# tsai0507/PolishPathPlanning

Hardware: AMD Instinct MI355X
Metric: polishing waypoints/sec for 1M-pt cloud, 256 slices; path L2 err vs ref (higher is better)
Workload: dtype f32; 1 GPU; cfg2_1m_s256; points_per_workpiece=999912, slices=256, waypoints_per_workpiece=25908, workpieces=1, batch_per_gpu=1, parallelism=single GPU, pairing=kd, walk=center_int (connect), dynamic_adjustment=False, handles_taking_turns=3

## Files before the change

polishpathplanning_amd/csrc/ppp_engine.hip:

```cpp
#include "ppp_kernels.h"
#ifdef PPP_SINGLE_TU
#include "ppp_window.h"
#else
#include "ppp_window_decl.h"
#endif
#include "ppp_preproc.h"
#include "ppp_sort.h"
#include "ppp_align.h"
#include "ppp_gather.h"
#include <atomic>
#include <cerrno>
#include <fcntl.h>
#include <thread>
#include <unistd.h>
#ifndef PPP_NN_HINT_SPACINGS
#define PPP_NN_HINT_SPACINGS 3.0
#endif
#ifndef PPP_SLAB_PTS
#define PPP_SLAB_PTS 832
#endif
#ifndef PPP_PPT8_FROM
#define PPP_PPT8_FROM 500000
#endif
#ifndef WIN_SLICE_WAVES_PER_CU
// ... 139 lines not shown
    DevBuf<int> wp_cnt, wp_off, tail, slice_wpcnt;
    DevBuf<float4> wp_xyz, wp_normal;
    DevBuf<int> wp_nn;
    DevBuf<float> wp_pre, wp_smooth, wp_out;
    DevBuf<MinMaxPart> mm_part;
    DevBuf<int> big_slabs, big_slices;
    DevBuf<char> arena;
    bool big_path = false;
    int mm_grid = 1, mm_grid_used = 1, sm_tiles = 1;
    DevBuf<char> scratch;
    bool win_allowed = true;
    bool win_disabled = false;
    bool win_path = false;
    bool win_staged = false;
    bool stage_compact = true;
    float win_pad = 4.f;
    int win_NBc_thr = 0;
    int win_capw = 0, win_cap_el = 0, win_NB = 0, win_NBc = 0, win_stride = 1, win_threads = 256, win_ppt = 4, win_gs = 1;
    int win_rec_lds = 0;
    int win_nkept = 0, win_first_kept = 0, win_el_expect = 0;
    float win_px0 = 0.f;
    DevBuf<float> win_px;
    DevBuf<int> win_cnt;
    DevBuf<float4> win_pts;
    DevBuf<MinMaxPart> win_part;
    DevBuf<float4> wps_xyz, wps_normal, wps_rec;
    DevBuf<int> fin_ticket;
    DevBuf<int> wps_nn;
    DevBuf<float> wps_pre;

// ... 417 lines not shown
    memset(&A, 0, sizeof(A));
    A.m = h->meta.p; A.P = dev_params(h);
    A.X = h->use_part ? h->Xp.p : h->X.p; A.Y = h->use_part ? h->Yp.p : h->Y.p; A.Z = h->use_part ? h->Zp.p : h->Z.p;
    A.idmap = h->use_part ? h->part_idx.p : ((h->part_given && h->part_has_idx) ? h->part_idx.p : nullptr);
    A.n = h->use_part ? h->n_part : (int)h->n;
    A.plan_px = h->win_px.p;
    A.S = h->S_cap; A.sb = h->sb; A.se = h->se; A.first_kept = h->win_first_kept; A.nkept = h->win_nkept;
    A.pad = h->win_pad; A.px0 = h->win_px0; A.inv_step = 1.0f / (float)std::max(1, (int)(h->P.tool_radius * 2));
    A.y0 = h->h_mn[1];
    { const float yr = h->h_mx[1] - h->h_mn[1]; A.yscale = yr > 0.f ? (float)h->win_NBc / yr : 0.f; }
    for (int d = 0; d < 3; ++d) { A.plan_mn[d] = h->h_mn[d]; A.plan_mx[d] = h->h_mx[d]; }
    A.plan_nvalid = h->h_nvalid;
    A.capw = h->win_capw; A.cap_el = h->win_cap_el; A.NB = h->win_NB; A.NBc = h->win_NBc; A.stride = h->win_stride; A.rec_lds = h->win_rec_lds;
    A.W_cap = h->W_cap; A.node_cap = h->node_cap;
    A.g_scatter = h->win_gs; A.g_slice = std::max(0, h->se - h->sb); A.g_finish = h->sm_tiles;
    A.finish = h->ranged ? 0 : 1;
    A.win_cnt = h->win_cnt.p; A.win_pts = h->win_pts.p; A.win_part = h->win_part.p;
    A.px = h->px.p; A.lo = h->lo.p; A.hi = h->hi.p;
    A.node_x = h->node_x.p; A.node_y = h->node_y.p; A.node_z = h->node_z.p;
    A.node_start = h->node_start.p; A.node_cnt = h->node_cnt.p; A.band_cnt = h->band_cnt.p;
    A.wp_cnt = h->wp_cnt.p; A.wp_off = h->wp_off.p; A.tail = h->tail.p;
    A.wps_xyz = h->wps_xyz.p; A.wps_normal = h->wps_normal.p; A.wps_nn = h->wps_nn.p; A.wps_pre = h->wps_pre.p; A.wps_rec = h->wps_rec.p;
    A.wp_pre = h->wp_pre.p; A.wp_smooth = h->wp_smooth.p; A.wp_out = h->wp_out.p; A.out2 = h->out2; A.out2_cap = h->out2_cap;
    A.plan_rec = (h->rec_current && h->plan_walk_ok) ? h->plan_auto.p : nullptr;
    A.meta_host = h->hmeta_pinned.p; A.fin_ticket = h->fin_ticket.p;
    return A;
}
size_t win_slice_lds(const ppp_handle h) { return win_slice_lds_for(h, h->win_NBc); }
void win_args_throughput(const ppp_handle h, WinArgs &A)
{
    A.NBc = h->win_NBc_thr; A.NB = WIN_CLASSES * A.NBc;
// ... 14 lines not shown
    else LAUNCH(h, "k_win_scatter", (k_win_scatter<4, false>), A.g_scatter, WSC_T, scat_lds, A);
    const int T = h->win_threads;
    const size_t lds = win_slice_lds_for(h, A.NBc);
    const int extra = tuning_env("PPP_WIN_NO_VERIFY") ? 0 : 1;
    if (T <= 256) LAUNCH(h, "k_win_slice", k_win_slice<256>, A.g_slice + extra, T, lds, A);
    else if (T <= 512) LAUNCH(h, "k_win_slice", k_win_slice<512>, A.g_slice + extra, T, lds, A);
    else if (T <= 768) LAUNCH(h, "k_win_slice", k_win_slice<768>, A.g_slice + extra, T, lds, A);
    else LAUNCH(h, "k_win_slice", k_win_slice<1024>, A.g_slice + extra, T, lds, A);
    h->stage_compact = false;
    return PPP_OK;
}
int enqueue_window_finish(ppp_handle h)
{
    const WinArgs A = win_args(h);
    LAUNCH(h, "k_win_finish", k_win_finish, A.g_finish, SMF_T, sizeof(int) * ((size_t)A.nkept + 2), A);
    return PPP_OK;
}

template <class Sel>
int compact(ppp_handle h, Sel &sel, int n, int *cnt, int *total, const std::function<int(int)> &sized = nullptr)
{
    const int nblocks = (n + COMPACT_CHUNK - 1) / COMPACT_CHUNK;
    LAUNCH(h, "k_compact_count", k_compact_count<Sel>, nblocks, 256, 0, sel, n, cnt);
    LAUNCH(h, "k_compact_scan", k_compact_scan, 1, 1024, 0, cnt, nblocks, total);
    if (sized) {
        int kept = 0;
        HIPCHK(h, hipMemcpyAsync(&kept, total, sizeof(int), hipMemcpyDeviceToHost, h->stream));
        HIPCHK(h, hipStreamSynchronize(h->stream));
        if (int rc = sized(kept)) return rc;
    }
// ... 114 lines not shown
        h->dyn_maxNB = (int)std::min(4.0e6, std::max(0.0, yr - 4) / (h->P.tool_radius / 4) + 4);
        h->dyn_maxNA = (int)std::min(4.0e6, yr / 5 + 4);
        h->node_cap = (int)std::min(2.0e9, (double)h->node_cap + (double)h->S_cap * h->dyn_maxNA);
        int rc = ensure_dynamic_buffers(h);
        if (rc) return rc;
    }
    HIPCHK(h, h->node_x.ensure(h->node_cap)); HIPCHK(h, h->node_y.ensure(h->node_cap)); HIPCHK(h, h->node_z.ensure(h->node_cap));
    HIPCHK(h, h->node_start.ensure(h->S_cap)); HIPCHK(h, h->node_cnt.ensure(h->S_cap)); HIPCHK(h, h->band_cnt.ensure(h->S_cap));
    HIPCHK(h, h->wp_cnt.ensure(h->S_cap)); HIPCHK(h, h->wp_off.ensure(h->S_cap + 1)); HIPCHK(h, h->tail.ensure(h->S_cap));
    HIPCHK(h, h->slice_wpcnt.ensure(h->S_cap));
    HIPCHK(h, h->wp_xyz.ensure(h->W_cap)); HIPCHK(h, h->wp_normal.ensure(h->W_cap)); HIPCHK(h, h->wp_nn.ensure(h->W_cap));
    HIPCHK(h, h->wp_pre.ensure(6 * (size_t)h->W_cap)); HIPCHK(h, h->wp_smooth.ensure(6 * (size_t)h->W_cap));
    HIPCHK(h, h->wp_out.ensure(6 * (size_t)h->W_cap));
    h->sm_tiles = smooth_tiles(h->W_cap);
    { int rcw = plan_window(h, S, per); if (rcw) return rcw; }
    h->stage_compact = true;
    h->planned = true;
    h->index_built = false; h->gen_done = false; h->meta_fresh = false; h->path_done = false; h->list_final = false;
    h->drop_graph();
    return PPP_OK;
}

int slice_threads(const ppp_handle h, long long slices_in_launch)
{
    const bool two_fit = 2 * (slice_kd_bytes(h->capb) + 1024) <= (size_t)h->max_lds;
    return (two_fit && slices_in_launch >= 2LL * h->num_cus) ? 512 : SLICE_KD_T;
}

int enqueue_index(ppp_handle h)
{
    const int n = h->use_part ? h->n_part : (int)h->n;
// ... 416 lines not shown
const char *ppp_version(void) { return PPP_VERSION_STR; }

int ppp_create(int device_id, ppp_handle *out)
{
    if (!out) return PPP_ERR_ARG;
    *out = nullptr;
    int count = 0;
    if (hipGetDeviceCount(&count) != hipSuccess || count <= 0) return PPP_ERR_NO_DEVICE;
    if (device_id < 0 || device_id >= count) return PPP_ERR_ARG;
    if (hipSetDevice(device_id) != hipSuccess) return PPP_ERR_HIP;
    ppp_handle h = new ppp_handle_s();
    h->device = device_id;
    ppp_default_params(&h->P);
    if (hipStreamCreateWithFlags(&h->stream, hipStreamNonBlocking) != hipSuccess) { delete h; return PPP_ERR_HIP; }
    if (h->meta.ensure(1) != hipSuccess) { delete h; return PPP_ERR_HIP; }
    if (hipMemset(h->meta.p, 0, sizeof(DevMeta)) != hipSuccess) { delete h; return PPP_ERR_HIP; }
    if (h->fin_ticket.ensure(1 + WIN_FIN_GROUPS) != hipSuccess || hipMemset(h->fin_ticket.p, 0, sizeof(int) * (1 + WIN_FIN_GROUPS)) != hipSuccess) { delete h; return PPP_ERR_HIP; }
    if (h->hmeta_pinned.ensure(1) != hipSuccess) { delete h; return PPP_ERR_HIP; }
    int lds = 0;
    if (hipDeviceGetAttribute(&lds, hipDeviceAttributeMaxSharedMemoryPerBlock, device_id) == hipSuccess && lds > 0) h->max_lds = lds;
    hipDeviceProp_t prop;
    if (hipGetDeviceProperties(&prop, device_id) == hipSuccess) {
        if (strncmp(prop.gcnArchName, "gfx950", 6) == 0) h->max_lds = std::max(h->max_lds, 160 * 1024);
        if (prop.multiProcessorCount > 0) h->num_cus = prop.multiProcessorCount;
    }
    (void)hipFuncSetAttribute((const void *)k_slice, hipFuncAttributeMaxDynamicSharedMemorySize, h->max_lds - 1024);
    (void)hipFuncSetAttribute((const void *)k_slice_kd<false>, hipFuncAttributeMaxDynamicSharedMemorySize, h->max_lds - 1024);
    (void)hipFuncSetAttribute((const void *)k_minmax<true>, hipFuncAttributeMaxDynamicSharedMemorySize, 16384 * 4);
    (void)hipFuncSetAttribute((const void *)k_slab_scatter<0, 4>, hipFuncAttributeMaxDynamicSharedMemorySize, 16384 * 4);
    (void)hipFuncSetAttribute((const void *)k_slab_scatter<0, 8>, hipFuncAttributeMaxDynamicSharedMemorySize, 16384 * 4);
    (void)hipFuncSetAttribute((const void *)k_slab_scatter<1, 8>, hipFuncAttributeMaxDynamicSharedMemorySize, 16384 * 4);
    (void)hipFuncSetAttribute((const void *)k_slab_scatter<2, 4>, hipFuncAttributeMaxDynamicSharedMemorySize, 16384 * 4);
// ... 633 lines not shown
               h->wp_xyz.p, h->wp_nn.p, h->wp_normal.p, h->wp_pre.p, PB, h->slab_ytab.p, cnt_in);
    } else
    {
#define PPP_POSE_ARGS h->meta.p, D, h->sorted4.p, h->slab_start.p, h->slab_xmin.p, \
           h->slab_xmax.p, h->px.p, h->node_x.p, h->node_y.p, h->node_z.p, h->node_start.p, h->node_cnt.p, h->wp_cnt.p, h->wp_off.p, \
           h->tail.p, h->W_cap, h->big_path ? 1 : 0, h->knot_cap, h->stage_cap, h->tab_slabs, h->pose_pad, \
           h->wp_xyz.p, h->wp_nn.p, h->wp_normal.p, h->wp_pre.p, PB, h->slab_ytab.p, cnt_in
        if (h->pose_threads <= 256) LAUNCH(h, "k_pose", (k_pose<false, 256>), nk, h->pose_threads, pose_lds_bytes(h->knot_cap, h->stage_cap, h->tab_slabs), PPP_POSE_ARGS);
        else if (h->pose_threads <= 512) LAUNCH(h, "k_pose", (k_pose<false, 512>), nk, h->pose_threads, pose_lds_bytes(h->knot_cap, h->stage_cap, h->tab_slabs), PPP_POSE_ARGS);
        else if (h->pose_threads <= 768) LAUNCH(h, "k_pose", (k_pose<false, 768>), nk, h->pose_threads, pose_lds_bytes(h->knot_cap, h->stage_cap, h->tab_slabs), PPP_POSE_ARGS);
        else LAUNCH(h, "k_pose", (k_pose<false, POSE_T>), nk, h->pose_threads, pose_lds_bytes(h->knot_cap, h->stage_cap, h->tab_slabs), PPP_POSE_ARGS);
#undef PPP_POSE_ARGS
    }
    h->path_done = true;
    h->list_final = false;
    h->stage_compact = true;
    if (!h->ranged) {
        int rc = enqueue_finish(h, D);
        if (rc) return rc;
        h->list_final = true;
        return PPP_OK;
    }
    return enqueue_meta_copy(h);
}

int ppp_finish_path_async(ppp_handle h, const float *pre6_dev, size_t W, const int *counts, size_t nkept)
{
    if (!h) return PPP_ERR_ARG;
    HIPCHK(h, hipSetDevice(h->device));
    { int rcs = settle(h); if (rcs) return rcs; }
    if (!h->have_cloud) return fail(h, PPP_ERR_ARG, "no cloud set");
    if (!h->planned) { int rc = make_plan(h); if (rc) return rc; }
    if ((W && !pre6_dev) || (nkept && !counts)) return fail(h, PPP_ERR_ARG, "bad arguments");
    if (W > (size_t)h->W_cap || nkept > (size_t)h->S_cap) return fail(h, PPP_ERR_CAPACITY, "the list is larger than this handle's plan (other cloud or parameters?)");
    if (!h->index_built && !h->win_path) { int rc = enqueue_index(h); if (rc) return rc; }
    DevParams D = dev_params(h);
    if (nkept) HIPCHK(h, hipMemcpyAsync(h->wp_cnt.p, counts, nkept * sizeof(int), hipMemcpyHostToDevice, h->stream));
    LAUNCH(h, "k_count_given", k_count_given, 1, 1024, 0, h->meta.p, D, (int)nkept, (int)W, h->wp_cnt.p, h->wp_off.p, h->tail.p, h->W_cap);
    if (W) LAUNCH(h, "k_load_pre", k_load_pre, (unsigned)((W + 255) / 256), 256, 0, h->meta.p, pre6_dev, h->wp_pre.p);
    int rc = enqueue_finish(h, D);
    if (rc) return rc;
    h->gen_done = true; ++h->gen_serial; h->path_done = true; h->list_final = true;
    h->stage_compact = true;
    return PPP_OK;
}

int ppp_run_async(ppp_handle h)
{
    if (!h) return PPP_ERR_ARG;
    HIPCHK(h, hipSetDevice(h->device));
    { int rcs = settle_enqueue_only(h); if (rcs) return rcs; }
    if (!h->have_cloud) return fail(h, PPP_ERR_ARG, "no cloud set");
    if (!h->planned) { int rc = make_plan(h); if (rc) return rc; }
    h->last_out2 = nullptr; h->last_out2_cap = 0;
    if (h->timing) {
        int rc = ppp_gen_path_async(h);
        return rc ? rc : ppp_get_path_async(h);
    }
// ... 15 lines not shown
        h->chain_calls = false;
        if (rc == PPP_OK) rc = ppp_get_path_async(h);
        --h->internal;
        hipGraph_t g = nullptr;
        hipError_t e = hipStreamEndCapture(h->stream, &g);
        if (rc != PPP_OK) { if (g) (void)hipGraphDestroy(g); return rc; }
        if (e != hipSuccess) return fail(h, PPP_ERR_HIP, std::string("hipStreamEndCapture: ") + hipGetErrorString(e));
        h->graph = g;
        e = hipGraphInstantiate(&h->graph_exec, h->graph, nullptr, nullptr, 0);
        if (e != hipSuccess) { h->drop_graph(); return fail(h, PPP_ERR_HIP, std::string("hipGraphInstantiate: ") + hipGetErrorString(e)); }
    }
    h->meta_fresh = false;
    HIPCHK(h, hipGraphLaunch(h->graph_exec, h->stream));
    if (!h->win_path) h->index_built = true;
    h->stage_compact = !h->win_path;
    h->gen_done = true; ++h->gen_serial; h->path_done = true;
    h->list_final = !h->ranged;
    h->meta_in_flight = true;
    h->meta_from_batch = false;
    return PPP_OK;
}

extern "C++" {
namespace {

bool batch_eligible(const ppp_handle h)
{
    return h->P.pairing == PPP_PAIR_KD && !h->P.dynamic_adjustment && !h->aligned && !h->ranged && !h->big_path && !h->two_pass_scatter &&
           slice_lds_ok(h, h->capb);
}
// ... 304 lines not shown
                return fail(lead, PPP_ERR_HIP, std::string("batch capture (") + where + "): " + hipGetErrorString(e != hipSuccess ? e : e2));
            }
            bg->g = g;
            e = hipGraphInstantiate(&bg->ge, bg->g, nullptr, nullptr, 0);
            if (e != hipSuccess) { discard(); return fail(lead, PPP_ERR_HIP, std::string("hipGraphInstantiate: ") + hipGetErrorString(e)); }
        }
        bg->epochs.resize(count);
        for (size_t i = 0; i < count; ++i) bg->epochs[i] = hs[i]->epoch;
    }
    if (bg->eager) { int rc = enqueue_batched(lead, bg); if (rc) return rc; }
    else HIPCHK(lead, hipGraphLaunch(bg->ge, lead->stream));
    for (size_t i = 0; i < count; ++i) {
        ppp_handle h = hs[i];
        if (!(bg->batched && bg->win) && !(!bg->batched && h->win_path)) h->index_built = true;
        h->stage_compact = !((bg->batched && bg->win) || (!bg->batched && h->win_path));
        h->gen_done = true; ++h->gen_serial; h->path_done = true;
        h->list_final = !h->ranged;
        h->meta_fresh = false;
        h->meta_in_flight = !(bg->batched && count == 1);
        h->meta_from_batch = bg->batched && count > 1;
        if (bg->batched && count > 1) { h->bmetas = bg->hmetas; h->bslot = i; }
        h->pending_stream = (i == 0) ? nullptr : lead->stream;
        remember_dst(i);
    }
    return PPP_OK;
}

extern "C++" {
namespace {
struct Rccl {
// ... 181 lines not shown
int ppp_get_waypoint_counts(ppp_handle h, int *counts, size_t cap, size_t *nkept)
{
    int rc = ensure_ready(h, true, true);
    if (rc) return rc;
    rc = map_dev_err(h);
    if (rc) return rc;
    size_t nk = (size_t)h->hmeta.nkept;
    if (nkept) *nkept = nk;
    if (counts && cap) {
        size_t k = std::min(cap, nk);
        if (k) HIPCHK(h, copy_sync(h, counts, h->wp_cnt.p, k * sizeof(int), hipMemcpyDeviceToHost));
    }
    return PPP_OK;
}

int ppp_copy_stage_to_device(ppp_handle h, int stage, float *dst_dev, size_t cap, size_t *W)
{
    int rc = ensure_ready(h, true, true);
    if (rc) return rc;
    rc = map_dev_err(h);
    if (rc) return rc;
    const float *src = stage == PPP_STAGE_WP_PRESMOOTH ? h->wp_pre.p : stage == PPP_STAGE_WP_SMOOTHED ? h->wp_smooth.p : nullptr;
    if (!src) return fail(h, PPP_ERR_ARG, "stage must be PPP_STAGE_WP_PRESMOOTH or PPP_STAGE_WP_SMOOTHED");
    if (stage == PPP_STAGE_WP_SMOOTHED && !h->list_final) return fail(h, PPP_ERR_ARG, NOT_FINAL_MSG);
    size_t w = (size_t)h->hmeta.W;
    if (W) *W = w;
    size_t k = std::min(cap, w);
    if (k && dst_dev) {
        HIPCHK(h, hipMemcpyAsync(dst_dev, src, k * 24, hipMemcpyDeviceToDevice, h->stream));
        HIPCHK(h, hipStreamSynchronize(h->stream));
    }
    return PPP_OK;
}

static int bounds_ready(ppp_handle h)
{
    if (h && h->have_cloud && h->planned && h->win_path && h->gen_done) {
        HIPCHK(h, hipSetDevice(h->device));
        return PPP_OK;
// ... 453 lines not shown
           h->slab_xmax.p, dq, (int)k, dout);
    HIPCHK(h, hipMemcpyAsync(idx, dout, k * 4, hipMemcpyDeviceToHost, h->stream));
    HIPCHK(h, hipStreamSynchronize(h->stream));
    return PPP_OK;
}

static int ensure_stage_lists(ppp_handle h)
{
    if (h->stage_compact || !h->win_path) return PPP_OK;
    const WinArgs A = win_args(h);
    if (A.nkept > 0) LAUNCH(h, "k_win_gather_stage", k_win_gather_stage, A.nkept, 256, 0, A, h->wp_xyz.p, h->wp_nn.p, h->wp_normal.p);
    h->stage_compact = true;
    return PPP_OK;
}

int ppp_get_stage(ppp_handle h, int stage, void *out, size_t cap_bytes, size_t *count)
{
    int rc = ensure_ready(h, true, true);
    if (rc) return rc;
    rc = map_dev_err(h);
    if (rc) return rc;
    if (stage == PPP_STAGE_WP_XYZ || stage == PPP_STAGE_WP_NN || stage == PPP_STAGE_WP_NORMAL) { rc = ensure_stage_lists(h); if (rc) return rc; }
    size_t W = (size_t)h->hmeta.W;
    if (count) *count = W;
    if (!out || !cap_bytes || !W) return PPP_OK;
    const void *src = nullptr;
    size_t elem = 0;
    std::vector<float> tmp;
    switch (stage) {
    case PPP_STAGE_WP_XYZ: {
        std::vector<float4> t4(W);
        HIPCHK(h, copy_sync(h, t4.data(), h->wp_xyz.p, W * 16, hipMemcpyDeviceToHost));
        tmp.resize(3 * W);
        for (size_t i = 0; i < W; ++i) { tmp[3 * i] = t4[i].x; tmp[3 * i + 1] = t4[i].y; tmp[3 * i + 2] = t4[i].z; }
        memcpy(out, tmp.data(), std::min(cap_bytes, W * 12));
        return PPP_OK;
    }
// ... 198 lines not shown
```

polishpathplanning_amd/csrc/ppp_window.h:

```cpp
#pragma once
#include "ppp_kernels.h"
#include "ppp_window_decl.h"

template <int PPT, bool STAGED>
__device__ __forceinline__ void win_scatter_body(const WinArgs &A, const int bx)
{
    extern __shared__ __attribute__((aligned(16))) int s_dyn[];
    float *s_px = (float *)s_dyn;
    int *s_cnt = s_dyn + A.S;
    __shared__ int s_scr[17];
    __shared__ float s_mn[3][WSC_T / 64], s_mx[3][WSC_T / 64];
    __shared__ int s_n[WSC_T / 64];
    const int S = A.S, n = A.n;
    const int i0 = bx * (PPT * (int)blockDim.x);
    STAMP_BEGIN();
    float4 p[PPT];
#pragma unroll
    for (int k = 0; k < PPT; ++k) {
        const int i = i0 + threadIdx.x + k * (int)blockDim.x;
        if (i < n) p[k] = make_float4(A.X[i], A.Y[i], A.Z[i], __int_as_float(A.idmap ? A.idmap[i] : i));
        else p[k] = make_float4(NAN, 0.f, 0.f, 0.f);
    }
    for (int s = threadIdx.x; s < S; s += blockDim.x) { s_px[s] = A.plan_px[s]; s_cnt[s] = 0; }
    if (bx == 0 && threadIdx.x == 0) {
        DevMeta *m = A.m;
        m->W = 0; m->err = 0; m->err_slice = 0x7fffffff; m->sweeps = 0; m->any_short = 0; m->rpy_oob = 0;
        m->node_cursor = 0; m->smooth_done = -1; m->emit_ticket = 0; m->big_slabs = 0; m->big_slices = 0; m->arena_cursor = 0; m->win_flag = 0;
        if (A.fin_ticket) for (int q = 0; q <= WIN_FIN_GROUPS; ++q) A.fin_ticket[q] = 0;
    }
    __syncthreads();
    STAMP(7, 0);
    float mn[3] = {INFINITY, INFINITY, INFINITY}, mx[3] = {-INFINITY, -INFINITY, -INFINITY};
    int cnt = 0;
    int pw[PPT], pr[PPT];
#pragma unroll
    for (int k = 0; k < PPT; ++k) {
        const float x = p[k].x;
        pw[k] = -1; pr[k] = 0;
        if (x == x) {
            mn[0] = fminf(mn[0], x); mx[0] = fmaxf(mx[0], x);
            mn[1] = fminf(mn[1], p[k].y); mx[1] = fmaxf(mx[1], p[k].y);
            mn[2] = fminf(mn[2], p[k].z); mx[2] = fmaxf(mx[2], p[k].z);
            cnt++;
            const float fj = fminf(fmaxf(floorf((x - s_px[0]) * A.inv_step + 0.5f), 0.f), (float)(S - 1));
            const int j = (int)fj;
            const int ja = j > 0 ? j - 1 : j, jb = j + 1 < S ? j + 1 : j;
            const float da = fabsf(x - s_px[ja]), dj = fabsf(x - s_px[j]), db = fabsf(x - s_px[jb]);
            int w = -1;
            if (dj <= A.pad) w = j; else if (da <= A.pad) w = ja; else if (db <= A.pad) w = jb;
            if (w >= A.sb && w < A.se) { pw[k] = w; pr[k] = atomicAdd(&s_cnt[w], 1); }
        }
    }
    __syncthreads();
    STAMP(7, 1);
    if (!STAGED) {
        for (int s = threadIdx.x; s < S; s += blockDim.x) {
            const int c = s_cnt[s];
            if (c) s_cnt[s] = atomicAdd(&A.win_cnt[(size_t)s * WIN_CNT_STRIDE], c);
        }
        __syncthreads();
        STAMP(7, 2);
#pragma unroll
        for (int k = 0; k < PPT; ++k) {
            if (pw[k] >= 0) {
                const int pos = s_cnt[pw[k]] + pr[k];
                if (pos < A.capw) A.win_pts[(size_t)pw[k] * A.capw + pos] = p[k];
            }
        }
    } else {
        int *s_loc = (int *)s_px;
        int *s_gb = s_dyn + 2 * S;
        float4 *stage = (float4 *)(s_dyn + ((3 * S + 3) & ~3));
        u16 *widx = (u16 *)(stage + PPT * (int)blockDim.x);
        int K;
        {
            const int per = (S + (int)blockDim.x - 1) / (int)blockDim.x;
            const int b0 = threadIdx.x * per;
            int sum = 0;
            for (int q = 0; q < per; ++q) if (b0 + q < S) sum += s_cnt[b0 + q];
            int pre = block_exscan_w(sum, s_scr, &K);
            for (int q = 0; q < per; ++q) {
                if (b0 + q < S) {
                    const int c = s_cnt[b0 + q];
                    s_loc[b0 + q] = pre; pre += c;
                    s_gb[b0 + q] = c ? atomicAdd(&A.win_cnt[(size_t)(b0 + q) * WIN_CNT_STRIDE], c) : 0;
                }
            }
        }
        __syncthreads();
#pragma unroll
        for (int k = 0; k < PPT; ++k) {
            if (pw[k] >= 0) {
                const int q = s_loc[pw[k]] + pr[k];
                stage[q] = p[k]; widx[q] = (u16)pw[k];
            }
        }
        __syncthreads();
        for (int q = threadIdx.x; q < K; q += blockDim.x) {
            const int w = widx[q];
            const int pos = s_gb[w] + (q - s_loc[w]);
            if (pos < A.capw) A.win_pts[(size_t)w * A.capw + pos] = stage[q];
        }
    }
    STAMP(7, 3);
    const int lane = threadIdx.x & 63, wid = threadIdx.x >> 6;
    for (int d = 0; d < 3; ++d) { mn[d] = wave_min(mn[d]); mx[d] = wave_max(mx[d]); }
    cnt = wave_sum(cnt);
    if (lane == 0) { for (int d = 0; d < 3; ++d) { s_mn[d][wid] = mn[d]; s_mx[d][wid] = mx[d]; } s_n[wid] = cnt; }
    __syncthreads();
    if (threadIdx.x == 0) {
        MinMaxPart r;
        r.cnt = 0; r.pad = 0;
        const int nw = (int)(blockDim.x >> 6);
        for (int w = 0; w < nw; ++w) r.cnt += s_n[w];
        for (int d = 0; d < 3; ++d) {
            float a = INFINITY, b = -INFINITY;
            for (int w = 0; w < nw; ++w) { a = fminf(a, s_mn[d][w]); b = fmaxf(b, s_mx[d][w]); }
            r.mn[d] = a; r.mx[d] = b;
        }
        A.win_part[bx] = r;
    }
    STAMP(7, 4);
}

__device__ __forceinline__ void win_lds_barrier() { asm volatile("s_waitcnt lgkmcnt(0)\n\ts_barrier" ::: "memory"); }

template <int PPT>
__device__ __forceinline__ void win_scatter_staged_loop(const WinArgs &A, const int bx, const int nwg)
{
    extern __shared__ __attribute__((aligned(16))) int s_dyn[];
    float *s_px = (float *)s_dyn;
    int *s_cnt = s_dyn + A.S;
    __shared__ int s_scr[17];
    __shared__ float s_mn[3][WSC_T / 64], s_mx[3][WSC_T / 64];
    __shared__ int s_n[WSC_T / 64];
// ... 795 lines not shown
    __syncthreads();
    const int S = s_S;
    int bad = 0;
    for (int s = tid; s < S; s += T) {
        const float v = s_px[s];
        if (v != A.plan_px[s]) bad = 1;
        const int position = (int)v;
        A.px[s] = v; A.lo[s] = (float)(-2 + position); A.hi[s] = (float)(2 + position);
    }
    if (bad) s_bad = 1;
    __syncthreads();
    if (tid == 0 && s_bad) win_flag(m, WIN_FLAG_STALE);
}

#define META_PUT(ptr, val) __hip_atomic_store((ptr), (val), __ATOMIC_RELAXED, __HIP_MEMORY_SCOPE_AGENT)
__device__ __forceinline__ void win_finish_body(const WinArgs &A, const int bx)
{
    extern __shared__ __attribute__((aligned(16))) int s_off[];
    __shared__ float s_x[3][SMF_M];
    __shared__ int s_scan[17];
    __shared__ int s_run, s_short, s_last, s_err;
    __shared__ double s_rp[SMF_END];
    __shared__ double s_e[2][3];
    DevMeta *m = A.m;
    const DevParams &P = A.P;
    const int nk = A.nkept, tid = (int)threadIdx.x;
    if (tid == 0) { s_err = m->err | m->win_flag; s_run = 0; s_short = 0; }
    __syncthreads();
    if (s_err) return;
    const int res_i = (int)P.rpy_resolution;
// ... 7 lines not shown
        int tot;
        const int pre = block_exscan_w(c2, s_scan, &tot);
        const int run = s_run;
        if (k2 < nk) {
            s_off[k2] = run + pre;
            if (P.rpy_resolution > 2 && c2 <= res_i) s_short = 1;
        }
        __syncthreads();
        if (tid == 0) s_run = run + tot;
        __syncthreads();
    }
    const int W = s_run;
    if (tid == 0) s_off[nk] = W;
    __syncthreads();
    if (W > A.W_cap) { if (bx == 0 && tid == 0) { set_err(m, DERR_CAPACITY, -1); META_PUT(&m->W, 0); } return; }
    if (bx == 0) {
        for (int k2 = tid; k2 < nk; k2 += blockDim.x) {
            A.wp_off[k2] = s_off[k2]; A.tail[k2] = s_off[k2 + 1] - 1;
            const int s2 = k2 + A.first_kept;
            if (s2 < A.sb || s2 >= A.se) A.wp_cnt[k2] = 0;
        }
        if (tid == 0) { A.wp_off[nk] = W; META_PUT(&m->W, W); META_PUT(&m->any_short, s_short); META_PUT(&m->sweeps, 0); META_PUT(&m->smooth_done, 0); }
    }
    const int ntiles = smooth_tiles(W);
    const int tile = bx;
    if (W == 0 || tile >= ntiles) return;
    auto slice_of = [&](int g) {
        int kk = (int)(((long long)g * (long long)nk) / (long long)W);
        kk = kk < 0 ? 0 : (kk > nk - 1 ? nk - 1 : kk);
        int steps = 0;
        while (kk > 0 && s_off[kk] > g && steps < 6) { --kk; ++steps; }
// ... 2 lines not shown
        return kk;
    };
    auto row_of = [&](int g) { const int kk = slice_of(g); return (size_t)kk * A.stride + (size_t)(g - s_off[kk]); };
    const double wd = 0.65, ws = 1 - wd, dg = wd + 2 * ws;
    const double r = (dg - sqrt(dg * dg - 4 * ws * ws)) / (2 * ws), c = wd / (dg - 2 * ws * r);
    const int t0 = tile * SMF_T;
    const int base = t0 - SMF_K;
    const bool solve = A.finish && P.smooth && W > 2;
    const int g = t0 + tid;
    int kk = 0;
    size_t rowbase = 0;
    float p[6] = {0.f, 0.f, 0.f, 0.f, 0.f, 0.f};
    if (g < W) {
        kk = slice_of(g);
        rowbase = (size_t)kk * A.stride - (size_t)s_off[kk];
#pragma unroll
        for (int d = 0; d < 6; ++d) p[d] = A.wps_pre[6 * (rowbase + g) + d];
    }
    if (A.finish) {
        const bool src = g >= 1 && g <= W - 2;
        for (int j = 0; j < 3; ++j) s_x[j][tid + SMF_K] = src ? p[j] : 0.f;
        if (tid < 2 * SMF_K) {
            const int l = tid < SMF_K ? tid : SMF_T + tid;
            const int g2 = base + l;
            const bool src2 = g2 >= 1 && g2 <= W - 2;
            size_t row = 0;
            if (src2) row = row_of(g2);
            for (int j = 0; j < 3; ++j) s_x[j][l] = src2 ? A.wps_pre[6 * row + j] : 0.f;
        }
    }
    const bool in_order = A.finish && P.rpy_resolution > 2 && s_short;
    const bool copy2 = A.finish && A.out2 != nullptr && W <= A.out2_cap;
    if (A.finish && A.out2 != nullptr && W > A.out2_cap && tile == 0 && tid == 0) set_err(m, DERR_CAPACITY, -1);
    const bool near_end = solve && (t0 < SMF_END || t0 + SMF_T - 1 > W - 1 - SMF_END);
    if (near_end) {
        if (tid < SMF_END) s_rp[tid] = smooth_rpow(r, tid);
        const int j = tid >> 6, lane = tid & 63;
        if (j < 3) {
            const int kq = (lane & 31) + 1;
            const int gq = lane < 32 ? kq : W - 1 - kq;
            double v = (gq >= 1 && gq <= W - 2) ? (double)A.wps_pre[6 * row_of(gq) + j] * smooth_rpow(r, kq) : 0.0;
            for (int o = 16; o > 0; o >>= 1) v += __shfl_xor(v, o, 64);
            if ((lane & 31) == 0) s_e[lane >> 5][j] = (double)A.wps_pre[6 * row_of(lane < 32 ? 0 : W - 1) + j] - c * v;
        }
    }
    __syncthreads();
    if (g < W) {
#pragma clang fp contract(on)
        for (int d = 0; d < 6; ++d) A.wp_pre[6 * (size_t)g + d] = p[d];
        if (A.finish) {
            if (solve) {
                const int l = g - base;
                double y[3];
#pragma unroll
                for (int j = 0; j < 3; ++j) {
                    double acc = (double)s_x[j][l - SMF_K] + (double)s_x[j][l + SMF_K];
#pragma unroll 8
                    for (int q = SMF_K - 1; q >= 1; --q) acc = ((double)s_x[j][l - q] + (double)s_x[j][l + q]) + r * acc;
                    y[j] = c * ((double)s_x[j][l] + r * acc);
                }
                if (near_end) {
                    const double D = W - 1 < SMF_END ? s_rp[W - 1] : 0.0;
                    const double r0 = g < SMF_END ? s_rp[g] : 0.0, r1 = W - 1 - g < SMF_END ? s_rp[W - 1 - g] : 0.0;
                    const double det = 1.0 - D * D;
#pragma unroll
                    for (int j = 0; j < 3; ++j) {
                        const double e0 = s_e[0][j], e1 = s_e[1][j];
                        const double Aa = (e0 - D * e1) / det, Bb = (e1 - D * e0) / det;
                        y[j] = y[j] + (Aa * r0 + Bb * r1);
                    }
                }
                if (g >= 1 && g <= W - 2) { p[0] = (float)y[0]; p[1] = (float)y[1]; p[2] = (float)y[2]; }
            }
            for (int d = 0; d < 6; ++d) A.wp_smooth[6 * (size_t)g + d] = p[d];
            if (!in_order) {
                if (P.rpy_resolution > 2) {
                    const int res = res_i;
                    const int p0 = s_off[kk], tl = s_off[kk + 1] - 1;
                    const int nfull = (tl - p0) / res;
                    const int lastkey = p0 + nfull * res;
                    const int rr = g - p0;
                    const float *src = A.wps_pre + 6 * rowbase;
                    if (g > lastkey) {
                        for (int D = 3; D < 6; ++D) p[D] = src[6 * (size_t)lastkey + D];
                    } else if (rr % res != 0) {
                        const int pre = p0 + (rr / res) * res, last = pre + res, wi = g - pre;
                        for (int D = 3; D < 6; D++) {
                            const float a = src[6 * (size_t)last + D], bb = src[6 * (size_t)pre + D];
                            double dr;
                            if (a * bb >= 0) {
                                dr = (double)((a - bb) / res);
                            } else {
                                double no1, no2;
                                if (a < 0) { no2 = bb; no1 = 2 * M_PI + a; }
                                else { no2 = 2 * M_PI + bb; no1 = a; }
                                dr = (double)fabsf(a - bb) < fabs(no1 - no2) ? (double)(a - bb) : (no1 - no2);
                                dr /= res;
                            }
                            float v = bb;
                            for (int q = 1; q <= wi; ++q) v = (float)(dr + v);
                            p[D] = v;
                        }
                    }
                    for (int D = 3; D < 6; ++D) p[D] = (double)p[D] > M_PI ? (float)((double)p[D] - 2 * M_PI) : p[D];
                }
                float R[3][3];
                rot_zyx(p[3], p[4], p[5], R);
                const float ee[3] = {0.f, 0.f, -P.ee_length};
                float t[3];
                for (int i = 0; i < 3; ++i) t[i] = R[i][0] * ee[0] + R[i][1] * ee[1] + R[i][2] * ee[2] + p[i] * 1.f;
                p[0] = t[0]; p[1] = t[1]; p[2] = t[2];
            }
            for (int d = 0; d < 6; ++d) A.wp_out[6 * (size_t)g + d] = p[d];
            if (copy2 && !in_order) for (int d = 0; d < 6; ++d) A.out2[6 * (size_t)g + d] = p[d];
        }
    }
    if (in_order) {
        __threadfence();
        __syncthreads();
        if (tid == 0) s_last = atomicAdd(&m->emit_ticket, 1) == ntiles - 1;
        __syncthreads();
        if (s_last) {
            __threadfence();
            if (tid == 0) { finish_list_in_order(m, P, A.tail, A.wp_out); m->emit_ticket = 0; }
            __threadfence();
            __syncthreads();
            if (copy2) for (size_t i = tid; i < 6 * (size_t)W; i += blockDim.x) A.out2[i] = A.wp_out[i];
        }
    }
// ... 100 lines not shown
        for (int i = threadIdx.x; i < 3 * S; i += blockDim.x) { census_host[i] = __hip_atomic_load(&cnt[i], __ATOMIC_RELAXED, __HIP_MEMORY_SCOPE_AGENT); cnt[i] = 0; }
        for (int i = threadIdx.x; i < S; i += blockDim.x) px_host[i] = px[i];
    }
    if (threadIdx.x == 0) {
        PlanAuto r = *plan;
        r.census = valid ? 1 : 0;
        *plan_host = r;
        *ticket = 0;
    }
}

template <int PPT, bool STAGED>
__global__ void __launch_bounds__(WSC_T) k_win_scatter(WinArgs A)
{
    if (STAGED) win_scatter_staged_loop<PPT>(A, blockIdx.x, A.g_scatter);
    else win_scatter_body<PPT, false>(A, blockIdx.x);
}
template <int PPT, bool STAGED>
__global__ void __launch_bounds__(WSC_T) k_win_scatter_b(const WinArgs *__restrict__ mem)
{
    const WinArgs &A = mem[blockIdx.y];
    if ((int)blockIdx.x >= A.g_scatter) return;
    if (STAGED) win_scatter_staged_loop<PPT>(A, blockIdx.x, A.g_scatter);
    else win_scatter_body<PPT, false>(A, blockIdx.x);
}
template <int TMAX>
__global__ void __launch_bounds__(TMAX) k_win_slice(WinArgs A)
{
    if ((int)blockIdx.x == A.g_slice) { win_verify_body(A); return; }
    win_slice_body<TMAX>(A, blockIdx.x);
}
template <int TMAX>
__global__ void __launch_bounds__(TMAX) k_win_slice_b(const WinArgs *__restrict__ mem)
{
    const WinArgs &A = mem[blockIdx.y];
    if ((int)blockIdx.x > A.g_slice) return;
    if ((int)blockIdx.x == A.g_slice) { win_verify_body(A); return; }
    win_slice_body<TMAX>(A, blockIdx.x);
}
// ... 41 lines not shown
```

polishpathplanning_amd/csrc/ppp_window_decl.h:

```cpp
#pragma once
#include "ppp_kernels.h"

enum { WIN_FLAG_OVERFLOW = 1,
       WIN_FLAG_REACH = 2,
       WIN_FLAG_STALE = 4 };
__device__ inline void win_flag(DevMeta *m, int why) { atomicOr(&m->win_flag, why); }

#define WIN_CLASSES 5
#ifndef WIN_CNT_STRIDE
#define WIN_CNT_STRIDE 1
#endif
#ifndef WIN_EMAX
#define WIN_EMAX 8
#endif
#ifndef WIN_CE
#define WIN_CE 4
#endif

struct WinArgs {
    DevMeta *m;
    DevParams P;
    const float *X, *Y, *Z;
    const int *idmap;
    int n;
    const float *plan_px;
    int S, sb, se, first_kept, nkept;
    float pad, px0, inv_step, y0, yscale;
    float plan_mn[3], plan_mx[3];
    int plan_nvalid;
    int capw, cap_el, NB, NBc, stride, W_cap, node_cap;
    int rec_lds;
    int g_scatter, g_slice, g_finish;
// ... 52 lines not shown
```

Baseline: 925.6 million waypoints/s.

## Defer smoothed-stage writes and restructure window scatter reductions and row I/O

The list-mode finish kernel stops writing wp_pre and wp_smooth intermediate buffers. They are regenerated lazily by a separate WIN_FIN_STAGES finish launch only when a caller asks for those stages, which removes global writes from the hot path. The scatter kernel now loads x/y/z separately with packed slot indices, delays the y/z min/max until after the global atomics, uses ds_swizzle wave folds, and builds the idmap-tagged float4 only at store time. Row loads and stores use float2 vector accesses. The handle init memsets are made async. The added cost is an extra kernel launch and state tracking for stage queries, and a risk of stale stage data if a flag is missed.

```diff
diff --git a/polishpathplanning_amd/csrc/ppp_engine.hip b/polishpathplanning_amd/csrc/ppp_engine.hip
--- a/polishpathplanning_amd/csrc/ppp_engine.hip
+++ b/polishpathplanning_amd/csrc/ppp_engine.hip
@@ -177,6 +177,7 @@
     bool win_path = false;
     bool win_staged = false;
     bool stage_compact = true;
+    bool stage_smooth = true;
     float win_pad = 4.f;
     int win_NBc_thr = 0;
     int win_capw = 0, win_cap_el = 0, win_NB = 0, win_NBc = 0, win_stride = 1, win_threads = 256, win_ppt = 4, win_gs = 1;
@@ -624,7 +625,7 @@
     A.capw = h->win_capw; A.cap_el = h->win_cap_el; A.NB = h->win_NB; A.NBc = h->win_NBc; A.stride = h->win_stride; A.rec_lds = h->win_rec_lds;
     A.W_cap = h->W_cap; A.node_cap = h->node_cap;
     A.g_scatter = h->win_gs; A.g_slice = std::max(0, h->se - h->sb); A.g_finish = h->sm_tiles;
-    A.finish = h->ranged ? 0 : 1;
+    A.finish = h->ranged ? WIN_FIN_RANGED : WIN_FIN_LIST;
     A.win_cnt = h->win_cnt.p; A.win_pts = h->win_pts.p; A.win_part = h->win_part.p;
     A.px = h->px.p; A.lo = h->lo.p; A.hi = h->hi.p;
     A.node_x = h->node_x.p; A.node_y = h->node_y.p; A.node_z = h->node_z.p;
@@ -669,6 +670,7 @@
 {
     const WinArgs A = win_args(h);
     LAUNCH(h, "k_win_finish", k_win_finish, A.g_finish, SMF_T, sizeof(int) * ((size_t)A.nkept + 2), A);
+    h->stage_smooth = A.finish != WIN_FIN_LIST;
     return PPP_OK;
 }
 
@@ -813,7 +815,7 @@
     HIPCHK(h, h->wp_out.ensure(6 * (size_t)h->W_cap));
     h->sm_tiles = smooth_tiles(h->W_cap);
     { int rcw = plan_window(h, S, per); if (rcw) return rcw; }
-    h->stage_compact = true;
+    h->stage_compact = true; h->stage_smooth = true;
     h->planned = true;
     h->index_built = false; h->gen_done = false; h->meta_fresh = false; h->path_done = false; h->list_final = false;
     h->drop_graph();
@@ -1260,8 +1262,9 @@
     ppp_default_params(&h->P);
     if (hipStreamCreateWithFlags(&h->stream, hipStreamNonBlocking) != hipSuccess) { delete h; return PPP_ERR_HIP; }
     if (h->meta.ensure(1) != hipSuccess) { delete h; return PPP_ERR_HIP; }
-    if (hipMemset(h->meta.p, 0, sizeof(DevMeta)) != hipSuccess) { delete h; return PPP_ERR_HIP; }
-    if (h->fin_ticket.ensure(1 + WIN_FIN_GROUPS) != hipSuccess || hipMemset(h->fin_ticket.p, 0, sizeof(int) * (1 + WIN_FIN_GROUPS)) != hipSuccess) { delete h; return PPP_ERR_HIP; }
+    if (hipMemsetAsync(h->meta.p, 0, sizeof(DevMeta), h->stream) != hipSuccess) { delete h; return PPP_ERR_HIP; }
+    if (h->fin_ticket.ensure(1 + WIN_FIN_GROUPS) != hipSuccess || hipMemsetAsync(h->fin_ticket.p, 0, sizeof(int) * (1 + WIN_FIN_GROUPS), h->stream) != hipSuccess) { delete h; return PPP_ERR_HIP; }
+    if (hipStreamSynchronize(h->stream) != hipSuccess) { delete h; return PPP_ERR_HIP; }
     if (h->hmeta_pinned.ensure(1) != hipSuccess) { delete h; return PPP_ERR_HIP; }
     int lds = 0;
     if (hipDeviceGetAttribute(&lds, hipDeviceAttributeMaxSharedMemoryPerBlock, device_id) == hipSuccess && lds > 0) h->max_lds = lds;
@@ -1925,7 +1928,7 @@
     }
     h->path_done = true;
     h->list_final = false;
-    h->stage_compact = true;
+    h->stage_compact = true; h->stage_smooth = true;
     if (!h->ranged) {
         int rc = enqueue_finish(h, D);
         if (rc) return rc;
@@ -1952,7 +1955,7 @@
     int rc = enqueue_finish(h, D);
     if (rc) return rc;
     h->gen_done = true; ++h->gen_serial; h->path_done = true; h->list_final = true;
-    h->stage_compact = true;
+    h->stage_compact = true; h->stage_smooth = true;
     return PPP_OK;
 }
 
@@ -1998,6 +2001,7 @@
     HIPCHK(h, hipGraphLaunch(h->graph_exec, h->stream));
     if (!h->win_path) h->index_built = true;
     h->stage_compact = !h->win_path;
+    h->stage_smooth = !h->win_path || h->ranged;
     h->gen_done = true; ++h->gen_serial; h->path_done = true;
     h->list_final = !h->ranged;
     h->meta_in_flight = true;
@@ -2332,6 +2336,7 @@
         ppp_handle h = hs[i];
         if (!(bg->batched && bg->win) && !(!bg->batched && h->win_path)) h->index_built = true;
         h->stage_compact = !((bg->batched && bg->win) || (!bg->batched && h->win_path));
+        h->stage_smooth = h->stage_compact || h->ranged;
         h->gen_done = true; ++h->gen_serial; h->path_done = true;
         h->list_final = !h->ranged;
         h->meta_fresh = false;
@@ -2543,6 +2548,7 @@
     return PPP_OK;
 }
 
+static int ensure_smooth_lists(ppp_handle h);
 int ppp_copy_stage_to_device(ppp_handle h, int stage, float *dst_dev, size_t cap, size_t *W)
 {
     int rc = ensure_ready(h, true, true);
@@ -2552,6 +2558,8 @@
     const float *src = stage == PPP_STAGE_WP_PRESMOOTH ? h->wp_pre.p : stage == PPP_STAGE_WP_SMOOTHED ? h->wp_smooth.p : nullptr;
     if (!src) return fail(h, PPP_ERR_ARG, "stage must be PPP_STAGE_WP_PRESMOOTH or PPP_STAGE_WP_SMOOTHED");
     if (stage == PPP_STAGE_WP_SMOOTHED && !h->list_final) return fail(h, PPP_ERR_ARG, NOT_FINAL_MSG);
+    rc = ensure_smooth_lists(h);
+    if (rc) return rc;
     size_t w = (size_t)h->hmeta.W;
     if (W) *W = w;
     size_t k = std::min(cap, w);
@@ -3035,6 +3043,16 @@
     return PPP_OK;
 }
 
+static int ensure_smooth_lists(ppp_handle h)
+{
+    if (h->stage_smooth || !h->win_path) return PPP_OK;
+    WinArgs A = win_args(h);
+    A.finish = WIN_FIN_STAGES; A.out2 = nullptr; A.out2_cap = 0; A.meta_host = nullptr;
+    LAUNCH(h, "k_win_finish", k_win_finish, A.g_finish, SMF_T, sizeof(int) * ((size_t)A.nkept + 2), A);
+    h->stage_smooth = true;
+    return PPP_OK;
+}
+
 int ppp_get_stage(ppp_handle h, int stage, void *out, size_t cap_bytes, size_t *count)
 {
     int rc = ensure_ready(h, true, true);
@@ -3042,6 +3060,7 @@
     rc = map_dev_err(h);
     if (rc) return rc;
     if (stage == PPP_STAGE_WP_XYZ || stage == PPP_STAGE_WP_NN || stage == PPP_STAGE_WP_NORMAL) { rc = ensure_stage_lists(h); if (rc) return rc; }
+    if (stage == PPP_STAGE_WP_PRESMOOTH || stage == PPP_STAGE_WP_SMOOTHED) { rc = ensure_smooth_lists(h); if (rc) return rc; }
     size_t W = (size_t)h->hmeta.W;
     if (count) *count = W;
     if (!out || !cap_bytes || !W) return PPP_OK;
diff --git a/polishpathplanning_amd/csrc/ppp_window.h b/polishpathplanning_amd/csrc/ppp_window.h
--- a/polishpathplanning_amd/csrc/ppp_window.h
+++ b/polishpathplanning_amd/csrc/ppp_window.h
@@ -2,26 +2,37 @@
 #include "ppp_kernels.h"
 #include "ppp_window_decl.h"
 
-template <int PPT, bool STAGED>
+#define WIN_SWZ(o) (0x1f | ((o) << 10))
+template <class Op>
+__device__ __forceinline__ float win_wave_fold(float v, Op op)
+{
+    v = op(v, __int_as_float(__builtin_amdgcn_ds_swizzle(__float_as_int(v), WIN_SWZ(16))));
+    v = op(v, __int_as_float(__builtin_amdgcn_ds_swizzle(__float_as_int(v), WIN_SWZ(8))));
+    v = op(v, __int_as_float(__builtin_amdgcn_ds_swizzle(__float_as_int(v), WIN_SWZ(4))));
+    v = op(v, __int_as_float(__builtin_amdgcn_ds_swizzle(__float_as_int(v), WIN_SWZ(2))));
+    v = op(v, __int_as_float(__builtin_amdgcn_ds_swizzle(__float_as_int(v), WIN_SWZ(1))));
+    return op(__int_as_float(__builtin_amdgcn_readlane(__float_as_int(v), 0)), __int_as_float(__builtin_amdgcn_readlane(__float_as_int(v), 32)));
+}
+
+template <int PPT>
 __device__ __forceinline__ void win_scatter_body(const WinArgs &A, const int bx)
 {
     extern __shared__ __attribute__((aligned(16))) int s_dyn[];
     float *s_px = (float *)s_dyn;
     int *s_cnt = s_dyn + A.S;
-    __shared__ int s_scr[17];
     __shared__ float s_mn[3][WSC_T / 64], s_mx[3][WSC_T / 64];
     __shared__ int s_n[WSC_T / 64];
-    const int S = A.S, n = A.n;
-    const int i0 = bx * (PPT * (int)blockDim.x);
+    const int S = A.S, n = A.n, T = (int)blockDim.x;
+    const int i0 = bx * (PPT * T);
     STAMP_BEGIN();
-    float4 p[PPT];
+    float px[PPT], py[PPT], pz[PPT];
 #pragma unroll
     for (int k = 0; k < PPT; ++k) {
-        const int i = i0 + threadIdx.x + k * (int)blockDim.x;
-        if (i < n) p[k] = make_float4(A.X[i], A.Y[i], A.Z[i], __int_as_float(A.idmap ? A.idmap[i] : i));
-        else p[k] = make_float4(NAN, 0.f, 0.f, 0.f);
-    }
-    for (int s = threadIdx.x; s < S; s += blockDim.x) { s_px[s] = A.plan_px[s]; s_cnt[s] = 0; }
+        const int i = i0 + (int)threadIdx.x + k * T;
+        if (i < n) { px[k] = A.X[i]; py[k] = A.Y[i]; pz[k] = A.Z[i]; }
+        else { px[k] = NAN; py[k] = 0.f; pz[k] = 0.f; }
+    }
+    for (int s = threadIdx.x; s < S; s += T) { s_px[s] = A.plan_px[s]; s_cnt[s] = 0; }
     if (bx == 0 && threadIdx.x == 0) {
         DevMeta *m = A.m;
         m->W = 0; m->err = 0; m->err_slice = 0x7fffffff; m->sweeps = 0; m->any_short = 0; m->rpy_oob = 0;
@@ -32,15 +43,13 @@
     STAMP(7, 0);
     float mn[3] = {INFINITY, INFINITY, INFINITY}, mx[3] = {-INFINITY, -INFINITY, -INFINITY};
     int cnt = 0;
-    int pw[PPT], pr[PPT];
+    int pk[PPT];
 #pragma unroll
     for (int k = 0; k < PPT; ++k) {
-        const float x = p[k].x;
-        pw[k] = -1; pr[k] = 0;
+        const float x = px[k];
+        pk[k] = -1;
         if (x == x) {
             mn[0] = fminf(mn[0], x); mx[0] = fmaxf(mx[0], x);
-            mn[1] = fminf(mn[1], p[k].y); mx[1] = fmaxf(mx[1], p[k].y);
-            mn[2] = fminf(mn[2], p[k].z); mx[2] = fmaxf(mx[2], p[k].z);
             cnt++;
             const float fj = fminf(fmaxf(floorf((x - s_px[0]) * A.inv_step + 0.5f), 0.f), (float)(S - 1));
             const int j = (int)fj;
@@ -48,77 +57,58 @@
             const float da = fabsf(x - s_px[ja]), dj = fabsf(x - s_px[j]), db = fabsf(x - s_px[jb]);
             int w = -1;
             if (dj <= A.pad) w = j; else if (da <= A.pad) w = ja; else if (db <= A.pad) w = jb;
-            if (w >= A.sb && w < A.se) { pw[k] = w; pr[k] = atomicAdd(&s_cnt[w], 1); }
+            if (w >= A.sb && w < A.se) pk[k] = (w << 16) | atomicAdd(&s_cnt[w], 1);
         }
     }
     __syncthreads();
     STAMP(7, 1);
-    if (!STAGED) {
-        for (int s = threadIdx.x; s < S; s += blockDim.x) {
-            const int c = s_cnt[s];
-            if (c) s_cnt[s] = atomicAdd(&A.win_cnt[(size_t)s * WIN_CNT_STRIDE], c);
-        }
-        __syncthreads();
-        STAMP(7, 2);
-#pragma unroll
-        for (int k = 0; k < PPT; ++k) {
-            if (pw[k] >= 0) {
-                const int pos = s_cnt[pw[k]] + pr[k];
-                if (pos < A.capw) A.win_pts[(size_t)pw[k] * A.capw + pos] = p[k];
-            }
-        }
-    } else {
-        int *s_loc = (int *)s_px;
-        int *s_gb = s_dyn + 2 * S;
-        float4 *stage = (float4 *)(s_dyn + ((3 * S + 3) & ~3));
-        u16 *widx = (u16 *)(stage + PPT * (int)blockDim.x);
-        int K;
-        {
-            const int per = (S + (int)blockDim.x - 1) / (int)blockDim.x;
-            const int b0 = threadIdx.x * per;
-            int sum = 0;
-            for (int q = 0; q < per; ++q) if (b0 + q < S) sum += s_cnt[b0 + q];
-            int pre = block_exscan_w(sum, s_scr, &K);
-            for (int q = 0; q < per; ++q) {
-                if (b0 + q < S) {
-                    const int c = s_cnt[b0 + q];
-                    s_loc[b0 + q] = pre; pre += c;
-                    s_gb[b0 + q] = c ? atomicAdd(&A.win_cnt[(size_t)(b0 + q) * WIN_CNT_STRIDE], c) : 0;
-                }
-            }
-        }
-        __syncthreads();
-#pragma unroll
-        for (int k = 0; k < PPT; ++k) {
-            if (pw[k] >= 0) {
-                const int q = s_loc[pw[k]] + pr[k];
-                stage[q] = p[k]; widx[q] = (u16)pw[k];
-            }
-        }
-        __syncthreads();
-        for (int q = threadIdx.x; q < K; q += blockDim.x) {
-            const int w = widx[q];
-            const int pos = s_gb[w] + (q - s_loc[w]);
-            if (pos < A.capw) A.win_pts[(size_t)w * A.capw + pos] = stage[q];
-        }
-    }
-    STAMP(7, 3);
+    const int s0 = (int)threadIdx.x;
+    const int c0 = s0 < S ? s_cnt[s0] : 0;
+    const int r0 = c0 ? atomicAdd(&A.win_cnt[(size_t)s0 * WIN_CNT_STRIDE], c0) : 0;
+    for (int s = s0 + T; s < S; s += T) {
+        const int c = s_cnt[s];
+        if (c) s_cnt[s] = atomicAdd(&A.win_cnt[(size_t)s * WIN_CNT_STRIDE], c);
+    }
+#pragma unroll
+    for (int k = 0; k < PPT; ++k) {
+        const bool ok = px[k] == px[k];
+        const float y = ok ? py[k] : NAN, z = ok ? pz[k] : NAN;
+        mn[1] = fminf(mn[1], y); mx[1] = fmaxf(mx[1], y);
+        mn[2] = fminf(mn[2], z); mx[2] = fmaxf(mx[2], z);
+    }
     const int lane = threadIdx.x & 63, wid = threadIdx.x >> 6;
-    for (int d = 0; d < 3; ++d) { mn[d] = wave_min(mn[d]); mx[d] = wave_max(mx[d]); }
-    cnt = wave_sum(cnt);
+    const auto fmin = [](float a, float b) { return fminf(a, b); };
+    const auto fmax = [](float a, float b) { return fmaxf(a, b); };
+    const auto isum = [](float a, float b) { return __int_as_float(__float_as_int(a) + __float_as_int(b)); };
+    for (int d = 0; d < 3; ++d) { mn[d] = win_wave_fold(mn[d], fmin); mx[d] = win_wave_fold(mx[d], fmax); }
+    cnt = __float_as_int(win_wave_fold(__int_as_float(cnt), isum));
     if (lane == 0) { for (int d = 0; d < 3; ++d) { s_mn[d][wid] = mn[d]; s_mx[d][wid] = mx[d]; } s_n[wid] = cnt; }
+    if (c0) s_cnt[s0] = r0;
+    STAMP(7, 2);
     __syncthreads();
     if (threadIdx.x == 0) {
         MinMaxPart r;
         r.cnt = 0; r.pad = 0;
-        const int nw = (int)(blockDim.x >> 6);
+        const int nw = T >> 6;
+#pragma unroll 1
         for (int w = 0; w < nw; ++w) r.cnt += s_n[w];
         for (int d = 0; d < 3; ++d) {
             float a = INFINITY, b = -INFINITY;
+#pragma unroll 1
             for (int w = 0; w < nw; ++w) { a = fminf(a, s_mn[d][w]); b = fmaxf(b, s_mx[d][w]); }
             r.mn[d] = a; r.mx[d] = b;
         }
         A.win_part[bx] = r;
+    }
+    STAMP(7, 3);
+#pragma unroll
+    for (int k = 0; k < PPT; ++k) {
+        if (pk[k] >= 0) {
+            const int w = pk[k] >> 16;
+            const int pos = s_cnt[w] + (pk[k] & 0xffff);
+            const int i = i0 + (int)threadIdx.x + k * T;
+            if (pos < A.capw) A.win_pts[(size_t)w * A.capw + pos] = make_float4(px[k], py[k], pz[k], __int_as_float(A.idmap ? A.idmap[i] : i));
+        }
     }
     STAMP(7, 4);
 }
@@ -944,6 +934,17 @@
 }
 
 #define META_PUT(ptr, val) __hip_atomic_store((ptr), (val), __ATOMIC_RELAXED, __HIP_MEMORY_SCOPE_AGENT)
+__device__ __forceinline__ void row_load(const float *__restrict__ src, float p[6])
+{
+    const float2 *q = (const float2 *)src;
+    const float2 a = q[0], b = q[1], c = q[2];
+    p[0] = a.x; p[1] = a.y; p[2] = b.x; p[3] = b.y; p[4] = c.x; p[5] = c.y;
+}
+__device__ __forceinline__ void row_store(float *dst, const float p[6])
+{
+    float2 *q = (float2 *)dst;
+    q[0] = make_float2(p[0], p[1]); q[1] = make_float2(p[2], p[3]); q[2] = make_float2(p[4], p[5]);
+}
 __device__ __forceinline__ void win_finish_body(const WinArgs &A, const int bx)
 {
     extern __shared__ __attribute__((aligned(16))) int s_off[];
@@ -981,7 +982,8 @@
     if (tid == 0) s_off[nk] = W;
     __syncthreads();
     if (W > A.W_cap) { if (bx == 0 && tid == 0) { set_err(m, DERR_CAPACITY, -1); META_PUT(&m->W, 0); } return; }
-    if (bx == 0) {
+    const bool stages = A.finish == WIN_FIN_STAGES;
+    if (bx == 0 && !stages) {
         for (int k2 = tid; k2 < nk; k2 += blockDim.x) {
             A.wp_off[k2] = s_off[k2]; A.tail[k2] = s_off[k2 + 1] - 1;
             const int s2 = k2 + A.first_kept;
@@ -1014,8 +1016,7 @@
     if (g < W) {
         kk = slice_of(g);
         rowbase = (size_t)kk * A.stride - (size_t)s_off[kk];
-#pragma unroll
-        for (int d = 0; d < 6; ++d) p[d] = A.wps_pre[6 * (rowbase + g) + d];
+        row_load(A.wps_pre + 6 * (rowbase + g), p);
     }
     if (A.finish) {
         const bool src = g >= 1 && g <= W - 2;
@@ -1029,9 +1030,10 @@
             for (int j = 0; j < 3; ++j) s_x[j][l] = src2 ? A.wps_pre[6 * row + j] : 0.f;
         }
     }
-    const bool in_order = A.finish && P.rpy_resolution > 2 && s_short;
-    const bool copy2 = A.finish && A.out2 != nullptr && W <= A.out2_cap;
-    if (A.finish && A.out2 != nullptr && W > A.out2_cap && tile == 0 && tid == 0) set_err(m, DERR_CAPACITY, -1);
+    const bool in_order = A.finish == WIN_FIN_LIST && P.rpy_resolution > 2 && s_short;
+    const bool copy2 = A.finish == WIN_FIN_LIST && A.out2 != nullptr && W <= A.out2_cap;
+    const bool vec2 = ((uintptr_t)A.out2 & 7) == 0;
+    if (A.finish == WIN_FIN_LIST && A.out2 != nullptr && W > A.out2_cap && tile == 0 && tid == 0) set_err(m, DERR_CAPACITY, -1);
     const bool near_end = solve && (t0 < SMF_END || t0 + SMF_T - 1 > W - 1 - SMF_END);
     if (near_end) {
         if (tid < SMF_END) s_rp[tid] = smooth_rpow(r, tid);
@@ -1047,7 +1049,7 @@
     __syncthreads();
     if (g < W) {
 #pragma clang fp contract(on)
-        for (int d = 0; d < 6; ++d) A.wp_pre[6 * (size_t)g + d] = p[d];
+        if (A.finish != WIN_FIN_LIST) row_store(A.wp_pre + 6 * (size_t)g, p);
         if (A.finish) {
             if (solve) {
                 const int l = g - base;
@@ -1072,7 +1074,7 @@
                 }
                 if (g >= 1 && g <= W - 2) { p[0] = (float)y[0]; p[1] = (float)y[1]; p[2] = (float)y[2]; }
             }
-            for (int d = 0; d < 6; ++d) A.wp_smooth[6 * (size_t)g + d] = p[d];
+            if (stages) { row_store(A.wp_smooth + 6 * (size_t)g, p); return; }
             if (!in_order) {
                 if (P.rpy_resolution > 2) {
                     const int res = res_i;
@@ -1082,7 +1084,9 @@
                     const int rr = g - p0;
                     const float *src = A.wps_pre + 6 * rowbase;
                     if (g > lastkey) {
-                        for (int D = 3; D < 6; ++D) p[D] = src[6 * (size_t)lastkey + D];
+                        const float2 *q = (const float2 *)(src + 6 * (size_t)lastkey);
+                        const float2 b = q[1], c = q[2];
+                        p[3] = b.y; p[4] = c.x; p[5] = c.y;
                     } else if (rr % res != 0) {
                         const int pre = p0 + (rr / res) * res, last = pre + res, wi = g - pre;
                         for (int D = 3; D < 6; D++) {
@@ -1111,8 +1115,11 @@
                 for (int i = 0; i < 3; ++i) t[i] = R[i][0] * ee[0] + R[i][1] * ee[1] + R[i][2] * ee[2] + p[i] * 1.f;
                 p[0] = t[0]; p[1] = t[1]; p[2] = t[2];
             }
-            for (int d = 0; d < 6; ++d) A.wp_out[6 * (size_t)g + d] = p[d];
-            if (copy2 && !in_order) for (int d = 0; d < 6; ++d) A.out2[6 * (size_t)g + d] = p[d];
+            row_store(A.wp_out + 6 * (size_t)g, p);
+            if (copy2 && !in_order) {
+                if (vec2) row_store(A.out2 + 6 * (size_t)g, p);
+                else for (int d = 0; d < 6; ++d) A.out2[6 * (size_t)g + d] = p[d];
+            }
         }
     }
     if (in_order) {
@@ -1243,7 +1250,7 @@
 __global__ void __launch_bounds__(WSC_T) k_win_scatter(WinArgs A)
 {
     if (STAGED) win_scatter_staged_loop<PPT>(A, blockIdx.x, A.g_scatter);
-    else win_scatter_body<PPT, false>(A, blockIdx.x);
+    else win_scatter_body<PPT>(A, blockIdx.x);
 }
 template <int PPT, bool STAGED>
 __global__ void __launch_bounds__(WSC_T) k_win_scatter_b(const WinArgs *__restrict__ mem)
@@ -1251,7 +1258,7 @@
     const WinArgs &A = mem[blockIdx.y];
     if ((int)blockIdx.x >= A.g_scatter) return;
     if (STAGED) win_scatter_staged_loop<PPT>(A, blockIdx.x, A.g_scatter);
-    else win_scatter_body<PPT, false>(A, blockIdx.x);
+    else win_scatter_body<PPT>(A, blockIdx.x);
 }
 template <int TMAX>
 __global__ void __launch_bounds__(TMAX) k_win_slice(WinArgs A)
diff --git a/polishpathplanning_amd/csrc/ppp_window_decl.h b/polishpathplanning_amd/csrc/ppp_window_decl.h
--- a/polishpathplanning_amd/csrc/ppp_window_decl.h
+++ b/polishpathplanning_amd/csrc/ppp_window_decl.h
@@ -16,6 +16,10 @@
 #ifndef WIN_CE
 #define WIN_CE 4
 #endif
+
+enum { WIN_FIN_RANGED = 0,
+       WIN_FIN_LIST = 1,
+       WIN_FIN_STAGES = 2   };
 
 struct WinArgs {
     DevMeta *m;
```

Result: faster. 969.5 million waypoints/s, median of 6 (+4.8%).
